# Ighina/MultimodalTopicSegmentation

Hardware: AMD Instinct MI355X
Metric: sentences/sec (fwd+bwd) (higher is better)
Workload: dtype bf16; 1 GPU; BASELINE configs[1]: restricted-window transformer tagger d=1792 heads=8 ff=256 radius=15 layers=1 focal loss, 64 docs x 256 sentences per GPU, fwd+bwd+Adam(eps 1e-7), inputs resident in HBM; global_batch_docs=64, sentences_per_doc=256, parallelism=dp1 (document-sharded, RCCL all-reduce)

## Files before the change

### multimodaltopicsegmentation_amd/csrc/ffn_fused.hip

```cpp
#include <algorithm>
#include "gemm_common.h"

#define FF_BM 64
#define FF_F 256
#define FF_IMG 32768
#define FF_RING (FF_IMG)
#define FF_A_STAGE (8192 + 32768)
#define FF_B_STAGE 32768
#define FF_LDS (FF_IMG + 4 * FF_B_STAGE)
#ifdef FFN_STAMPS
#define FSTAMP(i) do { const unsigned long long t_ = __builtin_amdgcn_s_memtime(); tacc[i] += t_ - tprev; tprev = t_; } while (0)
#else
#define FSTAMP(i) do { } while (0)
#endif

struct FfnArgs {
  const bf16_t* X;
  const bf16_t* Wa;
  const bf16_t* Wb;
  const float* ba;
  const float* bb;
  const bf16_t* U;
  bf16_t* Uout;
  bf16_t* T;
  bf16_t* Y;
  int M, D, relu;
#ifdef FFN_STAMPS
  unsigned long long* stamps;
#endif
};

__device__ __forceinline__ int ff_col(int j, int n) { return (j >> 1) * 32 + (n >> 2) * 8 + (j & 1) * 4 + (n & 3); }

template <bool PERM>
__device__ __forceinline__ void ff_piece_kmajor(const bf16_t* __restrict__ G, int ld, int row0, int dim, int k0, char* img, int piece, int lane) {
  const int row = piece * 8 + (lane >> 3), pos = lane & 7;
  const int ch = pos ^ ((row >> 1) & 7);
  const int srow = PERM ? (row & ~63) + ff_col((row >> 4) & 3, row & 15) : row;
  const bf16_t* src = G + (size_t)min(row0 + srow, dim - 1) * ld + k0 + ch * 8;
  __builtin_amdgcn_global_load_lds((gptr_t*)src, (lptr_t*)(img + piece * 1024), 16, 0, 0);
}
__device__ __forceinline__ void ff_piece_strided(const bf16_t* __restrict__ G, int ld, int k0, int col0, char* img, int piece, int lane) {
  const int kr = piece * 4 + (lane >> 4), c16 = lane & 15;
  const int ch = ((((c16 >> 1) ^ strided_key(kr))) << 1) | (c16 & 1);
  const bf16_t* src = G + (size_t)(k0 + kr) * ld + col0 + ch * 8;
  __builtin_amdgcn_global_load_lds((gptr_t*)src, (lptr_t*)(img + piece * 1024), 16, 0, 0);
}

__device__ __forceinline__ frag_raw ff_frag_strided(const char* tile, int kbase, int wcol0, int j, int lane) {
  const int r = lane & 15, q = r >> 2, p = r & 3;
  const int col = wcol0 + (j >> 1) * 32 + (j & 1) * 4 + 8 * p;
  const unsigned addr = (unsigned)(uintptr_t)(__attribute__((address_space(3))) const char*)(tile + strided_off(kbase + q, col));
  frag_raw f;
  asm volatile("ds_read_b64_tr_b16 %0, %1" : "=v"(f.lo) : "v"(addr));
  asm volatile("ds_read_b64_tr_b16 %0, %1 offset:1024" : "=v"(f.hi) : "v"(addr));
  return f;
}

#define FF_CWAVES 8
#define FF_LWAVES 4
#define FF_THREADS ((FF_CWAVES + FF_LWAVES) * 64)

template <bool BWD>
__global__ __launch_bounds__(FF_THREADS) void ffn_fused_kernel(const FfnArgs a) {
  constexpr bool WKM = !BWD;
  extern __shared__ __attribute__((aligned(16))) char smem[];
  char* fimg = smem;
  char* ring = smem + FF_RING;
  const int tid = threadIdx.x, lane = tid & 63;
  const int wave = __builtin_amdgcn_readfirstlane(tid >> 6);
  const int bm0 = blockIdx.x * FF_BM;
  const int D = a.D, M = a.M;
  const int nkA = D / 64, nch = D / 256, nB = nch * 4;
#ifdef FFN_STAMPS
  unsigned long long tacc[16] = {0, 0, 0, 0, 0, 0, 0, 0, 0, 0, 0, 0, 0, 0, 0, 0};
  unsigned long long tprev = __builtin_amdgcn_s_memtime();
#define FF_STAMPS_OUT() do { if (a.stamps && lane == 0) for (int i_ = 0; i_ < 16; ++i_) a.stamps[((size_t)blockIdx.x * 12 + wave) * 16 + i_] = tacc[i_]; } while (0)
#else
#define FF_STAMPS_OUT() do { } while (0)
#endif

  if (wave >= FF_CWAVES) {
    const int lw = wave - FF_CWAVES;
    auto dmaA = [&](int kt) {
      char* st = ring + (kt % 3) * FF_A_STAGE;
#pragma unroll
      for (int i = 0; i < 10; ++i) {
        const int q = lw * 10 + i;
        if (q < 8) ff_piece_kmajor<false>(a.X, D, bm0, M, kt * 64, st, q, lane);
        else if constexpr (WKM) ff_piece_kmajor<true>(a.Wa, D, 0, FF_F, kt * 64, st + 8192, q - 8, lane);
        else ff_piece_strided(a.Wa, FF_F, kt * 64, ((q - 8) >> 4) * 128, st + 8192 + ((q - 8) >> 4) * 16384, (q - 8) & 15, lane);
      }
    };
    auto dmaB = [&](int gi) {
      char* st = ring + (gi & 3) * FF_B_STAGE;
      const int c = gi >> 2, kk = gi & 3;
#pragma unroll
      for (int i = 0; i < 8; ++i) {
        const int q = lw * 8 + i;
        if constexpr (WKM) ff_piece_kmajor<true>(a.Wb, FF_F, c * 256, D, kk * 64, st, q, lane);
        else ff_piece_strided(a.Wb, D, kk * 64, c * 256 + (q >> 4) * 128, st + (q >> 4) * 16384, q & 15, lane);
      }
    };
    dmaA(0);
    if (nkA > 1) { dmaA(1); asm volatile("s_waitcnt vmcnt(10)" ::: "memory"); }
    else asm volatile("s_waitcnt vmcnt(0)" ::: "memory");
    __builtin_amdgcn_s_barrier();
#pragma clang loop unroll(disable)
    for (int kt = 0; kt < nkA; ++kt) {
      if (kt + 2 < nkA) { dmaA(kt + 2); FSTAMP(0); asm volatile("s_waitcnt vmcnt(10)" ::: "memory"); }
      else asm volatile("s_waitcnt vmcnt(0)" ::: "memory");
      FSTAMP(3);
      __builtin_amdgcn_s_barrier();
      FSTAMP(4);
    }
    dmaB(0);
    dmaB(1);
    dmaB(2);
    dmaB(3);
    FSTAMP(5);
    asm volatile("s_waitcnt vmcnt(0)" ::: "memory");
    __builtin_amdgcn_s_barrier();
    FSTAMP(6);
#pragma clang loop unroll(disable)
    for (int gi = 0; gi < nB; ++gi) {
      if (gi >= 1 && gi + 3 < nB) { dmaB(gi + 3); FSTAMP(8); asm volatile("s_waitcnt vmcnt(16)" ::: "memory"); }
      else asm volatile("s_waitcnt vmcnt(0)" ::: "memory");
      FSTAMP(11);
      __builtin_amdgcn_s_barrier();
      FSTAMP(12);
    }
    FF_STAMPS_OUT();
    return;
  }

  const int wm = wave >> 2, wn = wave & 3;
  const int r16 = lane & 15, g = lane >> 4;
#ifdef FFN_STAMPS
  int tb = 0;
#endif
  f32x4 acc[2][4];
#pragma unroll
  for (int i = 0; i < 2; ++i)
#pragma unroll
    for (int j = 0; j < 4; ++j) acc[i][j] = (f32x4){0.f, 0.f, 0.f, 0.f};

  const unsigned lds0 = (unsigned)(uintptr_t)(__attribute__((address_space(3))) char*)smem;
  unsigned lk[2];
#pragma unroll
  for (int ks = 0; ks < 2; ++ks) lk[ks] = lds0 + r16 * 128 + (((ks * 4 + g) ^ ((r16 >> 1) & 7)) << 4);
  auto mma_tile = [&](int Aoff, int Boff) {
    LFrag<true> fa[2][2];
    LFrag<WKM> fb[4][2];
#pragma unroll
    for (int ks = 0; ks < 2; ++ks) {
      const unsigned ab = lk[ks] + Aoff + wm * 4096, bb = lk[ks] + Boff + wn * 8192;
#pragma unroll
      for (int j = 0; j < 4; ++j) {
        if constexpr (WKM) asm volatile("ds_read_b128 %0, %1 offset:%2" : "=v"(fb[j][ks].k) : "v"(bb), "n"(j * 2048));
        else fb[j][ks].s = ff_frag_strided(smem + Boff + (wn >> 1) * 16384, ks * 32 + 8 * g, (wn & 1) * 64, j, lane);
      }
#pragma unroll
      for (int i = 0; i < 2; ++i) asm volatile("ds_read_b128 %0, %1 offset:%2" : "=v"(fa[i][ks].k) : "v"(ab), "n"(i * 2048));
    }
    lgkm_wait<0>();
    FSTAMP(tb + 1);
    __builtin_amdgcn_s_setprio(1);
#pragma unroll
    for (int ks = 0; ks < 2; ++ks) {
      bf16x8 vb[4];
#pragma unroll
      for (int j = 0; j < 4; ++j) vb[j] = lfrag_get<WKM>(fb[j][ks]);
#pragma unroll
      for (int i = 0; i < 2; ++i) {
        const bf16x8 va = lfrag_get<true>(fa[i][ks]);
#pragma unroll
        for (int j = 0; j < 4; ++j) acc[i][j] = __builtin_amdgcn_mfma_f32_16x16x32_bf16(vb[j], va, acc[i][j], 0, 0, 0);
      }
    }
    __builtin_amdgcn_s_setprio(0);
    FSTAMP(tb + 2);
  };

  typedef __attribute__((ext_vector_type(4))) unsigned u32x4;
  uint4 upre[2][2];
  float4 b1[2][2];
  if constexpr (BWD) {
#pragma unroll
    for (int i = 0; i < 2; ++i)
#pragma unroll
      for (int h = 0; h < 2; ++h)
        upre[i][h] = *reinterpret_cast<const uint4*>(a.U + (size_t)min(bm0 + wm * 32 + i * 16 + r16, M - 1) * FF_F + wn * 64 + h * 32 + g * 8);
  } else {
#pragma unroll
    for (int h = 0; h < 2; ++h)
#pragma unroll
      for (int e = 0; e < 2; ++e) b1[h][e] = *reinterpret_cast<const float4*>(a.ba + wn * 64 + h * 32 + g * 8 + e * 4);
  }
  __builtin_amdgcn_s_barrier();
#pragma clang loop unroll(disable)
  for (int kt = 0; kt < nkA; ++kt) {
    FSTAMP(0);
    const int st = FF_RING + (kt % 3) * FF_A_STAGE;
    mma_tile(st, st + 8192);
    FSTAMP(3);
    __builtin_amdgcn_s_barrier();
    FSTAMP(4);
  }
#pragma unroll
  for (int i = 0; i < 2; ++i) {
    const int row = wm * 32 + i * 16 + r16;
#pragma unroll
    for (int h = 0; h < 2; ++h) {
      float v[8];
#pragma unroll
      for (int e = 0; e < 4; ++e) { v[e] = acc[i][2 * h][e]; v[4 + e] = acc[i][2 * h + 1][e]; }
      const size_t go = (size_t)(bm0 + row) * FF_F + wn * 64 + h * 32 + g * 8;
      if constexpr (!BWD) {
        v[0] += b1[h][0].x; v[1] += b1[h][0].y; v[2] += b1[h][0].z; v[3] += b1[h][0].w;
        v[4] += b1[h][1].x; v[5] += b1[h][1].y; v[6] += b1[h][1].z; v[7] += b1[h][1].w;
        uint4 pre;
        pre.x = pack_bf16x2(v[0], v[1]); pre.y = pack_bf16x2(v[2], v[3]); pre.z = pack_bf16x2(v[4], v[5]); pre.w = pack_bf16x2(v[6], v[7]);
        *reinterpret_cast<uint4*>(a.Uout + go) = pre;
#pragma unroll
        for (int r = 0; r < 8; ++r) v[r] = a.relu ? fmaxf(v[r], 0.0f) : gelu_erf_f(v[r]);
      } else {
        const unsigned uw[4] = {upre[i][h].x, upre[i][h].y, upre[i][h].z, upre[i][h].w};
#pragma unroll
        for (int r = 0; r < 8; ++r) {
          const float uu = (r & 1) ? bf16_hi(uw[r >> 1]) : bf16_lo(uw[r >> 1]);
          const float dr = to_f32(from_f32<bf16_t>(v[r]));
          v[r] = a.relu ? (uu > 0.0f ? dr : 0.0f) : dr * gelu_erf_grad_f(uu);
        }
      }
      uint4 t;
      t.x = pack_bf16x2(v[0], v[1]); t.y = pack_bf16x2(v[2], v[3]); t.z = pack_bf16x2(v[4], v[5]); t.w = pack_bf16x2(v[6], v[7]);
      *reinterpret_cast<uint4*>(a.T + go) = t;
      *reinterpret_cast<uint4*>(fimg + wn * 8192 + kmajor_off(row, h * 4 + g)) = t;
    }
#pragma unroll
    for (int j = 0; j < 4; ++j) acc[i][j] = (f32x4){0.f, 0.f, 0.f, 0.f};
  }
  FSTAMP(5);
  asm volatile("s_waitcnt lgkmcnt(0)" ::: "memory");
  __builtin_amdgcn_s_barrier();
  FSTAMP(6);
#ifdef FFN_STAMPS
  tb = 8;
#endif

  float4 b2[2][2];
  uint4 res[2][2];
#pragma clang loop unroll(disable)
  for (int c = 0; c < nch; ++c) {
    const int colw = c * 256 + wn * 64 + g * 8;
#pragma unroll
    for (int kk = 0; kk < 4; ++kk) {
      const int gi = c * 4 + kk;
      if (kk == 3) {
        if constexpr (!BWD) {
#pragma unroll
          for (int h = 0; h < 2; ++h)
#pragma unroll
            for (int e = 0; e < 2; ++e) b2[h][e] = *reinterpret_cast<const float4*>(a.bb + colw + h * 32 + e * 4);
        }
      }
      if (kk == 1) {
#pragma unroll
        for (int i = 0; i < 2; ++i)
#pragma unroll
          for (int h = 0; h < 2; ++h)
            res[i][h] = *reinterpret_cast<const uint4*>(a.X + (size_t)min(bm0 + wm * 32 + i * 16 + r16, M - 1) * D + colw + h * 32);
      }
      FSTAMP(8);
      mma_tile(kk * 8192, FF_RING + kk * FF_B_STAGE);
      if (kk == 3) {
#pragma unroll
        for (int i = 0; i < 2; ++i) {
          const int row = bm0 + wm * 32 + i * 16 + r16;
#pragma unroll
          for (int h = 0; h < 2; ++h) {
            float v[8];
#pragma unroll
            for (int e = 0; e < 4; ++e) { v[e] = acc[i][2 * h][e]; v[4 + e] = acc[i][2 * h + 1][e]; }
            if constexpr (!BWD) {
              v[0] += b2[h][0].x; v[1] += b2[h][0].y; v[2] += b2[h][0].z; v[3] += b2[h][0].w;
              v[4] += b2[h][1].x; v[5] += b2[h][1].y; v[6] += b2[h][1].z; v[7] += b2[h][1].w;
            }
            const unsigned rw[4] = {res[i][h].x, res[i][h].y, res[i][h].z, res[i][h].w};
#pragma unroll
            for (int e = 0; e < 4; ++e) { v[2 * e] += bf16_lo(rw[e]); v[2 * e + 1] += bf16_hi(rw[e]); }
            uint4 o;
            o.x = pack_bf16x2(v[0], v[1]); o.y = pack_bf16x2(v[2], v[3]); o.z = pack_bf16x2(v[4], v[5]); o.w = pack_bf16x2(v[6], v[7]);
            *reinterpret_cast<uint4*>(a.Y + (size_t)row * D + colw + h * 32) = o;
          }
#pragma unroll
          for (int j = 0; j < 4; ++j) acc[i][j] = (f32x4){0.f, 0.f, 0.f, 0.f};
        }
      }
      FSTAMP(11);
      __builtin_amdgcn_s_barrier();
      FSTAMP(12);
    }
  }
  FF_STAMPS_OUT();
}

#ifdef FFN_STAMPS
static unsigned long long* g_ffn_stamps = nullptr;
extern "C" void mts_ffn_set_stamps(void* p) { g_ffn_stamps = (unsigned long long*)p; }
#endif
static int ffn_launch(bool bwd, hipStream_t st, const FfnArgs& a0) {
  FfnArgs a = a0;
#ifdef FFN_STAMPS
  a.stamps = g_ffn_stamps;
#endif
  const int grid = ceil_div(a.M, FF_BM);
  if (bwd) {
    auto k = ffn_fused_kernel<true>;
    if (int rc = mts_dyn_lds(k, FF_LDS, "ffn_fused")) return rc;
    hipLaunchKernelGGL(k, dim3(grid), dim3(FF_THREADS), FF_LDS, st, a);
  } else {
    auto k = ffn_fused_kernel<false>;
    if (int rc = mts_dyn_lds(k, FF_LDS, "ffn_fused")) return rc;
    hipLaunchKernelGGL(k, dim3(grid), dim3(FF_THREADS), FF_LDS, st, a);
  }
  MTS_LAUNCH_CHECK("mts_ffn_fused");
  return MTS_OK;
}

static int ffn_check(const char* who, int M, int D, int F, const void* p0, const void* p1, const void* p2, const void* p3, const void* p4) {
  MTS_CHECK_ARG(M > 0 && p0 && p1 && p2 && p3 && p4, "%s: bad arguments", who);
  MTS_UNSUPPORTED(F == FF_F && D >= 256 && D % 256 == 0, "%s: the fused block covers F = 256 and D a multiple of 256 (F=%d, D=%d)", who, F, D);
  return MTS_OK;
}

extern "C" int mts_ffn_supported(int dtype, int M, int D, int F) { return dtype == MTS_BF16 && M > 0 && F == FF_F && D >= 256 && D % 256 == 0; }

extern "C" int mts_ffn_fwd(void* stream, int M, int D, int F, const void* a1, const void* w1, const float* b1, const void* w2, const float* b2,
                           int relu, void* u, void* f, void* s2) {
  if (int rc = ffn_check("mts_ffn_fwd", M, D, F, a1, w1, w2, s2, f)) return rc;
  MTS_CHECK_ARG(b1 && b2 && u, "mts_ffn_fwd: null bias / u");
  FfnArgs a{(const bf16_t*)a1, (const bf16_t*)w1, (const bf16_t*)w2, b1, b2, nullptr, (bf16_t*)u, (bf16_t*)f, (bf16_t*)s2, M, D, relu};
  return ffn_launch(false, (hipStream_t)stream, a);
}

extern "C" int mts_ffn_bwd_data(void* stream, int M, int D, int F, const void* ds2, const void* w1, const void* w2, const void* u, int relu,
                                void* du, void* da1) {
  if (int rc = ffn_check("mts_ffn_bwd_data", M, D, F, ds2, w1, w2, du, da1)) return rc;
  MTS_CHECK_ARG(u, "mts_ffn_bwd_data: null u");
  FfnArgs a{(const bf16_t*)ds2, (const bf16_t*)w2, (const bf16_t*)w1, nullptr, nullptr, (const bf16_t*)u, nullptr, (bf16_t*)du, (bf16_t*)da1, M, D, relu};
  return ffn_launch(true, (hipStream_t)stream, a);
}
```

### multimodaltopicsegmentation_amd/csrc/gemm.hip

```cpp
#include <algorithm>
#include <math.h>
#include <stdlib.h>
#include "common.h"

#include "gemm_common.h"


template <int LAYOUT, typename TC, bool GLDS>
__global__ __launch_bounds__(256, 2) void gemm_bf16_kernel(const GemmArgs a) {
  constexpr bool A_KMAJOR = (LAYOUT == MTS_NT || LAYOUT == MTS_NN);
  constexpr bool B_KMAJOR = (LAYOUT == MTS_NT || LAYOUT == MTS_TT);
  extern __shared__ __attribute__((aligned(16))) char smem[];

  const int tid = threadIdx.x;
  const int lane = tid & 63;
  const int wave = tid >> 6;
  const int wm = wave >> 1, wn = wave & 1;
  const int r16 = lane & 15, g = lane >> 4;

  const int ntn = (a.N + BN - 1) / BN;
  const int ntm = (a.M + BM - 1) / BM;
  const int nt = ntn * ntm;
  int bid = xcd_remap(blockIdx.x, nt);
  const int bm0 = (ntm < ntn ? bid % ntm : bid / ntn) * BM;
// ... 329 lines not shown
      float v[4] = {0.f, 0.f, 0.f, 0.f};
      if (kc) {
        const int row = r0 + (f >> 2), k = k0 + (f & 3) * 4;
        if (row < rdim) {
          const float* p = X + (long)row * sr + k;
          if (vec && k + 3 < kend) { const float4 t = *reinterpret_cast<const float4*>(p); v[0] = t.x; v[1] = t.y; v[2] = t.z; v[3] = t.w; }
          else for (int j = 0; j < 4; ++j) if (k + j < kend) v[j] = p[j];
        }
      } else {
        const int k = k0 + (f >> 5), row = r0 + (f & 31) * 4;
        if (k < kend) {
          const float* p = X + (long)k * sk + row;
          if (vec && row + 3 < rdim) { const float4 t = *reinterpret_cast<const float4*>(p); v[0] = t.x; v[1] = t.y; v[2] = t.z; v[3] = t.w; }
          else for (int j = 0; j < 4; ++j) if (row + j < rdim) v[j] = p[j];
        }
      }
      r[i] = make_float4(v[0], v[1], v[2], v[3]);
    }
  };
  auto store_op = [&](float (&S)[F32_BK][F32_PITCH], bool kc, const float4 (&r)[2]) {
#pragma unroll
    for (int i = 0; i < 2; ++i) {
      const int f = tid + 256 * i;
      if (kc) {
        const int row = f >> 2, k = (f & 3) * 4;
        S[k][row] = r[i].x; S[k + 1][row] = r[i].y; S[k + 2][row] = r[i].z; S[k + 3][row] = r[i].w;
      } else {
        *reinterpret_cast<float4*>(&S[f >> 5][(f & 31) * 4]) = r[i];
      }
    }
  };

  f32x4 acc[4][4];
#pragma unroll
  for (int i = 0; i < 4; ++i)
#pragma unroll
    for (int j = 0; j < 4; ++j) acc[i][j] = (f32x4){0.f, 0.f, 0.f, 0.f};

  const int nk = (kend - kbeg + F32_BK - 1) / F32_BK;
  load_op(A, s.sam, s.sak, a_kc, a_vec, bm0, a.M, kbeg, ra);
  load_op(B, s.sbn, s.sbk, b_kc, b_vec, bn0, a.N, kbeg, rb);
  store_op(As[0], a_kc, ra);
  store_op(Bs[0], b_kc, rb);
  __syncthreads();
  for (int kt = 0; kt < nk; ++kt) {
    const int buf = kt & 1;
    if (kt + 1 < nk) {
      load_op(A, s.sam, s.sak, a_kc, a_vec, bm0, a.M, kbeg + (kt + 1) * F32_BK, ra);
      load_op(B, s.sbn, s.sbk, b_kc, b_vec, bn0, a.N, kbeg + (kt + 1) * F32_BK, rb);
    }
#pragma unroll
    for (int ks = 0; ks < F32_BK / 4; ++ks) {
      float av[4], bv[4];
#pragma unroll
      for (int i = 0; i < 4; ++i) {
        av[i] = As[buf][ks * 4 + g][wm * 64 + i * 16 + r16];
        bv[i] = Bs[buf][ks * 4 + g][wn * 64 + i * 16 + r16];
      }
#pragma unroll
      for (int i = 0; i < 4; ++i)
#pragma unroll
        for (int j = 0; j < 4; ++j) acc[i][j] = __builtin_amdgcn_mfma_f32_16x16x4f32(bv[j], av[i], acc[i][j], 0, 0, 0);
    }
    if (kt + 1 < nk) {
      store_op(As[buf ^ 1], a_kc, ra);
      store_op(Bs[buf ^ 1], b_kc, rb);
    }
    __syncthreads();
  }
#pragma unroll
  for (int i = 0; i < 4; ++i) {
    const int m = bm0 + wm * 64 + i * 16 + r16;
#pragma unroll
    for (int j = 0; j < 4; ++j) {
      const int n = bn0 + wn * 64 + j * 16 + 4 * g;
      float v[4] = {acc[i][j][0], acc[i][j][1], acc[i][j][2], acc[i][j][3]};
      epilogue4<float, float>(a, m, n, v, true);
    }
  }
}

#define COLSUM_RS 128
template <typename T>
__global__ __launch_bounds__(256) void colsum_partial_kernel(const T* __restrict__ X, int M, int N, int ldx,
                                                             float* __restrict__ partial) {
  __shared__ float red[16][64];
  const int cx = threadIdx.x & 15, ry = threadIdx.x >> 4;
  const int n = blockIdx.x * 64 + cx * 4;
  const int rs = blockIdx.y;
  const int rows_per = (M + COLSUM_RS - 1) / COLSUM_RS;
  const int m0 = rs * rows_per, m1 = min(M, m0 + rows_per);
  float s[4] = {0.f, 0.f, 0.f, 0.f};
  if (n + 3 < N) {
    int m = m0 + ry;
    for (; m + 48 < m1; m += 64) {
      float v[4][4];
#pragma unroll
      for (int u = 0; u < 4; ++u) load4<T>(X + (size_t)(m + 16 * u) * ldx + n, v[u]);
#pragma unroll
      for (int u = 0; u < 4; ++u)
#pragma unroll
        for (int i = 0; i < 4; ++i) s[i] += v[u][i];
    }
    for (; m < m1; m += 16) {
      float v[4];
      load4<T>(X + (size_t)m * ldx + n, v);
#pragma unroll
      for (int i = 0; i < 4; ++i) s[i] += v[i];
    }
  } else if (n < N) {
    for (int m = m0 + ry; m < m1; m += 16)
      for (int i = 0; i < 4 && n + i < N; ++i) s[i] += to_f32(X[(size_t)m * ldx + n + i]);
  }
#pragma unroll
  for (int i = 0; i < 4; ++i) red[ry][cx * 4 + i] = s[i];
  __syncthreads();
  if (threadIdx.x < 64) {
    const int c = threadIdx.x, nn = blockIdx.x * 64 + c;
    float t = 0.f;
#pragma unroll
    for (int r = 0; r < 16; ++r) t += red[r][c];
    if (nn < N) partial[(size_t)rs * N + nn] = t;
  }
}
__global__ __launch_bounds__(256) void colsum_final_kernel(const float* __restrict__ partial, int N, int nparts,
                                                           float* __restrict__ out, int accumulate) {
  __shared__ float red[4][64];
  const int col = threadIdx.x & 63, grp = threadIdx.x >> 6;
  const int n = blockIdx.x * 64 + col;
  float s = 0.f;
  if (n < N) {
    int r = grp;
    for (; r + 4 * 7 < nparts; r += 4 * 8) {
      float v[8];
#pragma unroll
      for (int u = 0; u < 8; ++u) v[u] = partial[(size_t)(r + 4 * u) * N + n];
#pragma unroll
      for (int u = 0; u < 8; ++u) s += v[u];
    }
    for (; r < nparts; r += 4) s += partial[(size_t)r * N + n];
  }
  red[grp][col] = s;
  __syncthreads();
  if (grp == 0 && n < N) {
    const float t = (red[0][col] + red[1][col]) + (red[2][col] + red[3][col]);
    out[n] = accumulate ? out[n] + t : t;
  }
}

__global__ __launch_bounds__(256) void splitk_reduce_kernel(const float* __restrict__ slab, int splits, int M, int N, float* __restrict__ C,
                                                            int ldc, int accumulate) {
  const size_t idx = (size_t)blockIdx.x * 256 + threadIdx.x;
  const int n4 = N / 4;
  if (idx >= (size_t)M * n4) return;
  const int m = (int)(idx / n4), n = 4 * (int)(idx % n4);
  float s[4] = {0.f, 0.f, 0.f, 0.f};
  if (accumulate) load4<float>(C + (size_t)m * ldc + n, s);
  const size_t plane = (size_t)M * N;
  for (int z = 0; z < splits; ++z) {
    float v[4];
    load4<float>(slab + z * plane + (size_t)m * N + n, v);
#pragma unroll
    for (int i = 0; i < 4; ++i) s[i] += v[i];
  }
  store4<float>(C + (size_t)m * ldc + n, s);
}

__global__ __launch_bounds__(256) void splitk_reduce_t_kernel(const float* __restrict__ slab, int splits, int M, int N, float* __restrict__ Ct,
                                                              int ldc, int accumulate) {
  __shared__ float tile[32][33];
  const int n0 = blockIdx.x * 32, m0 = blockIdx.y * 32;
  const int tx = threadIdx.x & 31, ty = threadIdx.x >> 5;
  const size_t plane = (size_t)M * N;
#pragma unroll
  for (int r = ty; r < 32; r += 8) {
    const int m = m0 + r, n = n0 + tx;
    float s = 0.f;
    if (m < M && n < N) {
      const float* p = slab + (size_t)m * N + n;
      int z = 0;
      for (; z + 7 < splits; z += 8) {
        float v[8];
#pragma unroll
        for (int u = 0; u < 8; ++u) v[u] = p[(size_t)(z + u) * plane];
#pragma unroll
        for (int u = 0; u < 8; ++u) s += v[u];
      }
      for (; z < splits; ++z) s += p[(size_t)z * plane];
    }
    tile[r][tx] = s;
  }
  __syncthreads();
#pragma unroll
  for (int r = ty; r < 32; r += 8) {
    const int n = n0 + r, m = m0 + tx;
    if (n < N && m < M) {
      float* o = Ct + (size_t)n * ldc + m;
      *o = accumulate ? *o + tile[tx][r] : tile[tx][r];
    }
  }
}

template <typename T> __global__ void cast_kernel(const float* __restrict__ src, T* __restrict__ dst, size_t n) {
  size_t i = ((size_t)blockIdx.x * blockDim.x + threadIdx.x) * 4;
  const size_t stride = (size_t)gridDim.x * blockDim.x * 4;
  for (; i + 3 < n; i += stride) {
    float v[4];
    load4<float>(src + i, v);
    store4<T>(dst + i, v);
  }
  if (i < n && i + 3 >= n)
    for (size_t j = i; j < n; ++j) dst[j] = from_f32<T>(src[j]);
}

template <typename T> __global__ void cast_concat_kernel(const float* __restrict__ s1, const float* __restrict__ s2, T* __restrict__ dst,
                                                          size_t rows, int D1, int D2) {
  const int D = D1 + D2, q = D / 4;
  const size_t total = rows * q;
  for (size_t i = (size_t)blockIdx.x * blockDim.x + threadIdx.x; i < total; i += (size_t)gridDim.x * blockDim.x) {
    const size_t r = i / q;
    const int e = (int)(i - r * q) * 4;
    float v[4];
    load4<float>(e < D1 ? s1 + r * D1 + e : s2 + r * D2 + (e - D1), v);
    store4<T>(dst + r * D + e, v);
  }
}

extern "C" int mts_cast_concat(void* stream, int dst_dtype, size_t rows, int D1, int D2, const float* src1, const float* src2, void* dst) {
  MTS_CHECK_ARG(src1 && src2 && dst && D1 > 0 && D2 > 0 && D1 % 4 == 0 && D2 % 4 == 0, "mts_cast_concat: bad arguments (widths must be multiples of 4)");
  if (rows == 0) return MTS_OK;
  const int blocks = (int)std::min<size_t>(4096, (rows * ((D1 + D2) / 4) + 255) / 256);
  if (dst_dtype == MTS_BF16) hipLaunchKernelGGL(cast_concat_kernel<bf16_t>, dim3(blocks), dim3(256), 0, (hipStream_t)stream, src1, src2, (bf16_t*)dst, rows, D1, D2);
  else if (dst_dtype == MTS_F32) hipLaunchKernelGGL(cast_concat_kernel<float>, dim3(blocks), dim3(256), 0, (hipStream_t)stream, src1, src2, (float*)dst, rows, D1, D2);
  else { mts_set_error("mts_cast_concat: bad dtype %d", dst_dtype); return MTS_ERR_INVALID; }
  MTS_LAUNCH_CHECK("mts_cast_concat");
  return MTS_OK;
}

extern "C" size_t mts_colsum_workspace(int N) { return (size_t)COLSUM_RS * (size_t)N * sizeof(float); }

extern "C" int mts_colsum(void* stream, int dtype, int M, int N, const void* X, int ldx, float* out, int accumulate,
                          void* partial) {
  MTS_CHECK_ARG(M > 0 && N > 0 && X && out && partial, "mts_colsum: bad arguments");
  MTS_CHECK_ARG(dtype == MTS_F32 || dtype == MTS_BF16, "mts_colsum: bad dtype %d", dtype);
  MTS_CHECK_ARG(ldx % 4 == 0, "mts_colsum: ldx must be a multiple of 4");
  hipStream_t st = (hipStream_t)stream;
  const int nparts = min(COLSUM_RS, M);
  dim3 grid(ceil_div(N, 64), COLSUM_RS);
  (void)nparts;
  if (dtype == MTS_F32)
    hipLaunchKernelGGL(colsum_partial_kernel<float>, grid, dim3(256), 0, st, (const float*)X, M, N, ldx, (float*)partial);
  else
    hipLaunchKernelGGL(colsum_partial_kernel<bf16_t>, grid, dim3(256), 0, st, (const bf16_t*)X, M, N, ldx, (float*)partial);
  hipLaunchKernelGGL(colsum_final_kernel, dim3(ceil_div(N, 64)), dim3(256), 0, st, (const float*)partial, N, COLSUM_RS, out,
                     accumulate);
  MTS_LAUNCH_CHECK("mts_colsum");
  return MTS_OK;
}

extern "C" int mts_cast(void* stream, int dst_dtype, const float* src, void* dst, size_t n) {
  MTS_CHECK_ARG(src && dst, "mts_cast: null pointer");
  if (n == 0) return MTS_OK;
  hipStream_t st = (hipStream_t)stream;
  const int blocks = (int)std::min<size_t>(2048, (n / 4 + 255) / 256 + 1);
  if (dst_dtype == MTS_BF16)
    hipLaunchKernelGGL(cast_kernel<bf16_t>, dim3(blocks), dim3(256), 0, st, src, (bf16_t*)dst, n);
  else if (dst_dtype == MTS_F32)
    hipLaunchKernelGGL(cast_kernel<float>, dim3(blocks), dim3(256), 0, st, src, (float*)dst, n);
  else {
    mts_set_error("mts_cast: bad dtype %d", dst_dtype);
    return MTS_ERR_INVALID;
  }
  MTS_LAUNCH_CHECK("mts_cast");
  return MTS_OK;
}

int mts_launch_gemm256(const GemmArgs& a, int layout, bool c_is_f32, int splits, hipStream_t st);
int mts_launch_gemm224(const GemmArgs& a, int layout, bool c_is_f32, int splits, hipStream_t st);
bool mts_gemm224t_applies(const GemmArgs& a, int layout, bool c_is_f32, int splits);

static thread_local int g_gemm_glds = -1;
static thread_local int g_tile_mode = -1;
static thread_local int g_force_splits = 0;
static thread_local int g_tile_order = 1;
static thread_local int g_gemm_deep = 1;
static thread_local int g_chain = 0;
static thread_local int g_combine = 0;
#define MTS_GEMM_WS_HEAD 8192
static thread_local int g_last_tile = 0, g_last_splits = 0;

static thread_local void (*g_mid_hook)(void) = nullptr;
extern "C" int mts_gemm_set_mid_hook(void (*fn)(void)) { g_mid_hook = fn; return MTS_OK; }

extern "C" int mts_gemm_last_plan(int* tile, int* splits) {
  if (tile) *tile = g_last_tile;
  if (splits) *splits = g_last_splits;
  return MTS_OK;
}

void mts_band_set_mfma(int on);
void mts_band_set_fused(int on);
void mts_full_set_mfma(int on);
void mts_t5_set_mfma(int on);
static thread_local int g_f32_mfma = 1;
static thread_local int g_big_min_k = 256;
static thread_local int g_gemm_variant = 0;
void mts_lstm_pair_set_spin_limit(int n);
void mts_lstm_pair_set_max_pairs(int n);
void mts_lstm_pair_set_parts(int n);
extern "C" int mts_set_option(const char* key, int value) {
  if (!key) return MTS_ERR_INVALID;
  if (!strcmp(key, "gemm_tile")) { g_tile_mode = value; return MTS_OK; }
  if (!strcmp(key, "gemm_glds")) { g_gemm_glds = value; return MTS_OK; }
  if (!strcmp(key, "gemm_splits")) { g_force_splits = value; return MTS_OK; }
  if (!strcmp(key, "gemm_order")) { g_tile_order = value; return MTS_OK; }
  if (!strcmp(key, "gemm_chain")) { g_chain = value; return MTS_OK; }
  if (!strcmp(key, "gemm_combine")) { g_combine = value; return MTS_OK; }
  if (!strcmp(key, "gemm_deep")) { g_gemm_deep = value; return MTS_OK; }
  if (!strcmp(key, "gemm_variant")) { g_gemm_variant = value; return MTS_OK; }
  if (!strcmp(key, "gemm_big_min_k")) { g_big_min_k = value; return MTS_OK; }
  if (!strcmp(key, "gemm_f32_mfma")) { g_f32_mfma = value; return MTS_OK; }
  if (!strcmp(key, "band_mfma")) { mts_band_set_mfma(value); return MTS_OK; }
  if (!strcmp(key, "band_fused_bwd")) { mts_band_set_fused(value); return MTS_OK; }
  if (!strcmp(key, "full_mfma")) { mts_full_set_mfma(value); return MTS_OK; }
  if (!strcmp(key, "t5_mfma")) { mts_t5_set_mfma(value); return MTS_OK; }
  if (!strcmp(key, "lstm_pair_spin_limit")) { mts_lstm_pair_set_spin_limit(value); return MTS_OK; }
  if (!strcmp(key, "lstm_pair_max_pairs")) { mts_lstm_pair_set_max_pairs(value); return MTS_OK; }
  if (!strcmp(key, "lstm_parts")) { mts_lstm_pair_set_parts(value); return MTS_OK; }
  mts_set_error("mts_set_option: unknown key %s", key);
  return MTS_ERR_INVALID;
}

template <int LAYOUT, typename TC>
static void launch_bf16(const GemmArgs& a, int splits, hipStream_t st) {
  const int nt = ceil_div(a.M, BM) * ceil_div(a.N, BN);
  if (g_gemm_glds < 0) {
    const char* e = getenv("MTS_GEMM_GLDS");
    g_gemm_glds = (e && e[0] == '0') ? 0 : 1;
  }
  const bool glds = g_gemm_glds && (a.K % BK == 0) && (a.ksplit % BK == 0) && a.M >= 8 && a.N >= 8;
  if (glds) {
    GemmArgs b = a;
    const bool deep = g_gemm_deep && (size_t)nt * splits <= 256 && a.ksplit >= 4 * BK;
    b.nbuf = deep ? 4 : 2;
    auto k = gemm_bf16_kernel<LAYOUT, TC, true>;
    if (deep && mts_dyn_lds(k, 8 * TILE_BYTES, "gemm") != MTS_OK) b.nbuf = 2;
    hipLaunchKernelGGL(k, dim3(nt, 1, splits), dim3(256), (b.nbuf == 4 ? 8 : 4) * TILE_BYTES, st, b);
  } else {
    hipLaunchKernelGGL((gemm_bf16_kernel<LAYOUT, TC, false>), dim3(nt, 1, splits), dim3(256), 4 * TILE_BYTES, st, a);
  }
}

static void plan_bf16(int c_dtype, int layout, int M, int N, int K, unsigned epilogue, bool has_workspace, size_t workspace_bytes,
                      int* use256_out, int* splits_out) {
  if (g_tile_mode < 0) {
    const char* e = getenv("MTS_GEMM_TILE");
    g_tile_mode = e ? atoi(e) : 0;
  }
  const int tile_mode = g_tile_mode;
  const unsigned plain = epilogue & ~MTS_EPI_ACCUM;
  const bool can_split = (c_dtype == MTS_F32 && plain == 0 && has_workspace && N % 4 == 0 && K >= 2048);
  const bool can256 = (K % BK == 0) && K >= g_big_min_k && M >= 8 && N >= 8 && tile_mode != 128;
  const double bw = 3500.0;
  double best = 1e30;
  int splits = 1;
  int use256 = 0;
  const bool can224 = can256 && (N % 224 == 0) && tile_mode != 256;
  for (int big = 0; big <= (can256 ? 2 : 0); ++big) {
    if (big == 2 && !can224) continue;
    if (tile_mode == 256 && can256 && big != 1) continue;
    if (tile_mode == 224 && can224 && big != 2) continue;
    const int tile = big ? 256 : 128;
    const double slots = big ? 256.0 : 512.0;
    const double t_k = layout == MTS_TN ? (big == 2 ? (M % 256 == 0 ? 0.0160 : 0.0200) : big == 1 ? 0.0218 : 0.0145)
                                        : (big ? 0.0232 * (big == 2 ? 0.875 : 1.0) : 0.0180);
    const double t_0 = big ? 7.7 : 6.5;
    const int nt = ceil_div(M, tile) * (big == 2 ? N / 224 : ceil_div(N, tile));
    for (int sp = 1; sp <= (can_split ? 32 : 1); ++sp) {
      const int ks = ceil_div(ceil_div(K, sp), BK) * BK;
      if (ceil_div(K, ks) != sp) continue;
      if (sp > 1 && (size_t)sp * M * N * sizeof(float) > workspace_bytes) break;
      if (g_force_splits > 0 && can_split && sp != g_force_splits) continue;
      const double rounds = ceil((double)nt * sp / slots);
      const double cost = rounds * (ks * t_k + t_0) + (sp > 1 ? (2.0 * sp + 1.0) * M * N * 4.0 / 1e6 / bw : 0.0);
      if (cost < best) { best = cost; splits = sp; use256 = big; }
    }
  }
  *use256_out = use256;
  *splits_out = splits;
}

int mts_gemm224_last_kernel();
int mts_launch_gemm224t_pair(const GemmArgs& a, int splits, const void* A2, const void* B2, float* slab2, hipStream_t st);
bool mts_gemm224t_applies(const GemmArgs& a, int layout, bool c_is_f32, int splits);

static int wgrad_pair_splits(int M, int N, int K, size_t workspace_bytes) {
  if (M % 256 || N % 224 || K % 64 || K < 256) return -1;
  static int cus = 0;
  if (!cus) { int dev = 0; hipDeviceProp_t pr; cus = (hipGetDevice(&dev) == hipSuccess && hipGetDeviceProperties(&pr, dev) == hipSuccess) ? pr.multiProcessorCount : 256; }
  const int nt = (M / 256) * (N / 224);
  int sp = std::max(1, std::min(32, cus / (2 * nt)));
  for (; sp >= 1; --sp) {
    const int ks = ceil_div(ceil_div(K, sp), BK) * BK;
    if (ceil_div(K, ks) != sp) continue;
    if (ks >= 128 && K - (sp - 1) * ks >= 128 && (size_t)2 * sp * M * N * sizeof(float) <= workspace_bytes) return sp;
  }
  return -1;
}
extern "C" size_t mts_wgrad_pair_workspace(int M, int N, int K) {
  const int sp = wgrad_pair_splits(M, N, K, (size_t)-1);
  return sp < 1 ? 0 : (size_t)2 * sp * M * N * sizeof(float);
}
extern "C" int mts_wgrad_pair(void* stream, int M, int N, int K, const void* A1, const void* B1, float* C1, int ldc1, const void* A2, const void* B2,
                              float* C2t, int ldc2t, int lda, int ldb, int accumulate, void* workspace, size_t workspace_bytes) {
  MTS_CHECK_ARG(M > 0 && N > 0 && K > 0 && A1 && B1 && C1 && A2 && B2 && C2t && workspace, "mts_wgrad_pair: bad arguments");
  MTS_CHECK_ARG(ldc1 >= N && ldc2t >= M && ldc1 % 4 == 0, "mts_wgrad_pair: bad output strides");
  const int sp = wgrad_pair_splits(M, N, K, workspace_bytes);
  MTS_UNSUPPORTED(sp >= 1, "mts_wgrad_pair: M=%d N=%d K=%d not covered (M %% 256, N %% 224, K %% 64) or workspace too small", M, N, K);
  hipStream_t st = (hipStream_t)stream;
  GemmArgs a;
  memset(&a, 0, sizeof(a));
  a.A = A1; a.B = B1; a.C = C1;
  a.M = M; a.N = N; a.K = K; a.lda = lda; a.ldb = ldb; a.ldc = ldc1;
  a.epi = 0; a.colscale = 1.0f;
  a.ksplit = ceil_div(ceil_div(K, sp), BK) * BK;
  a.order = 1; a.nbuf = 2; a.variant = 0;
  float* const planes = (float*)workspace;
  a.slab = planes;
  float* const planes2 = planes + (size_t)sp * M * N;
  MTS_UNSUPPORTED(mts_gemm224t_applies(a, MTS_TN, true, sp), "mts_wgrad_pair: operands not covered by the four-wave weight-gradient kernel (alignment / strides)");
  const int rc = mts_launch_gemm224t_pair(a, sp, A2, B2, planes2, st);
  MTS_UNSUPPORTED(rc == MTS_OK, "mts_wgrad_pair: launch refused");
  hipLaunchKernelGGL(splitk_reduce_kernel, dim3((unsigned)(((size_t)M * (N / 4) + 255) / 256)), dim3(256), 0, st, (const float*)planes, sp, M, N, C1, ldc1,
                     accumulate ? 1 : 0);
  hipLaunchKernelGGL(splitk_reduce_t_kernel, dim3(ceil_div(N, 32), ceil_div(M, 32)), dim3(256), 0, st, (const float*)planes2, sp, M, N, C2t, ldc2t,
                     accumulate ? 1 : 0);
  MTS_LAUNCH_CHECK("mts_wgrad_pair");
  return MTS_OK;
}

extern "C" int mts_gemm_plan(int a_dtype, int c_dtype, int layout, int M, int N, int K, unsigned epilogue, size_t workspace_bytes,
                             int* tile, int* splits) {
  MTS_CHECK_ARG(M > 0 && N > 0 && K > 0, "mts_gemm_plan: bad shape M=%d N=%d K=%d", M, N, K);
  MTS_CHECK_ARG(layout == MTS_NT || layout == MTS_NN || layout == MTS_TN || layout == MTS_TT, "mts_gemm_plan: bad layout %d", layout);
  MTS_CHECK_ARG(a_dtype == MTS_F32 || a_dtype == MTS_BF16, "mts_gemm_plan: bad a_dtype %d", a_dtype);
  int use256 = 0, sp = 1;
  const size_t ws_planes = workspace_bytes > MTS_GEMM_WS_HEAD ? workspace_bytes - MTS_GEMM_WS_HEAD : 0;
  if (a_dtype == MTS_BF16) plan_bf16(c_dtype, layout, M, N, K, epilogue, ws_planes > 0, ws_planes, &use256, &sp);
  if (tile) *tile = a_dtype == MTS_F32 ? (g_f32_mfma ? 128 : 64) : use256 == 2 ? 224 : use256 == 1 ? 256 : 128;
  if (splits) *splits = sp;
  return MTS_OK;
}

extern "C" int mts_gemm(void* stream, int a_dtype, int c_dtype, int layout, int M, int N, int K, const void* A, int lda,
                        const void* B, int ldb, void* C, int ldc, const float* bias, const void* residual, int ldr,
                        void* aux, int ldaux, unsigned epilogue, float colscale, int ncols_scaled, void* workspace, size_t workspace_bytes) {
  MTS_CHECK_ARG(M > 0 && N > 0 && K > 0, "mts_gemm: bad shape M=%d N=%d K=%d", M, N, K);
  MTS_CHECK_ARG(A && B && C, "mts_gemm: null operand");
  MTS_CHECK_ARG(layout == MTS_NT || layout == MTS_NN || layout == MTS_TN || layout == MTS_TT, "mts_gemm: bad layout %d", layout);
  MTS_CHECK_ARG(a_dtype == MTS_F32 || a_dtype == MTS_BF16, "mts_gemm: bad a_dtype %d", a_dtype);
  MTS_CHECK_ARG(c_dtype == MTS_F32 || c_dtype == a_dtype, "mts_gemm: c_dtype must be f32 or a_dtype");
  MTS_CHECK_ARG(!(epilogue & MTS_EPI_BIAS) || bias, "mts_gemm: MTS_EPI_BIAS without bias");
  MTS_CHECK_ARG(!(epilogue & MTS_EPI_RESIDUAL) || residual, "mts_gemm: MTS_EPI_RESIDUAL without residual");
  MTS_CHECK_ARG(!(epilogue & MTS_EPI_ACCUM) || c_dtype == MTS_F32, "mts_gemm: MTS_EPI_ACCUM needs fp32 C");
  MTS_CHECK_ARG((epilogue & (MTS_EPI_GELU | MTS_EPI_RELU)) != (MTS_EPI_GELU | MTS_EPI_RELU), "mts_gemm: MTS_EPI_GELU and MTS_EPI_RELU are exclusive");
  hipStream_t st = (hipStream_t)stream;
  GemmArgs a;
  a.A = A; a.B = B; a.C = C; a.bias = bias; a.residual = residual; a.aux = aux;
  a.M = M; a.N = N; a.K = K; a.lda = lda; a.ldb = ldb; a.ldc = ldc; a.ldr = ldr; a.ldaux = ldaux;
  a.epi = epilogue; a.colscale = colscale; a.ncols_scaled = ncols_scaled;
  a.variant = g_gemm_variant;
#ifdef MTS_GEMM_STAMPS
  a.stamps = nullptr;
#endif
  a.ksplit = K; a.slab = nullptr; a.chain = nullptr; a.order = g_tile_order; a.nbuf = 2;

  if (a_dtype == MTS_F32) {
    StrideArgs s;
    if (layout == MTS_NT) { s.sam = lda; s.sak = 1; s.sbn = ldb; s.sbk = 1; }
    else if (layout == MTS_NN) { s.sam = lda; s.sak = 1; s.sbn = 1; s.sbk = ldb; }
    else if (layout == MTS_TT) { s.sam = 1; s.sak = lda; s.sbn = ldb; s.sbk = 1; }
    else { s.sam = 1; s.sak = lda; s.sbn = 1; s.sbk = ldb; }
    MTS_CHECK_ARG(ldc % 4 == 0 && ((uintptr_t)C % 16) == 0, "mts_gemm(f32): C must be 16-byte aligned with ldc %% 4 == 0");
    MTS_CHECK_ARG(!(epilogue & MTS_EPI_RESIDUAL) || (ldr % 4 == 0 && ((uintptr_t)residual % 16) == 0), "mts_gemm(f32): residual must be 16-byte aligned with ldr %% 4 == 0");
    MTS_CHECK_ARG(!aux || (ldaux % 4 == 0 && ((uintptr_t)aux % 16) == 0), "mts_gemm(f32): aux must be 16-byte aligned with ldaux %% 4 == 0");
    const int nt = ceil_div(M, F32_BM) * ceil_div(N, F32_BM);
    int splits = 1;
    if (g_f32_mfma && workspace && !(epilogue & ~MTS_EPI_ACCUM) && N % 4 == 0 && nt <= 128 && K >= 1024) {
      splits = std::min(std::min(16, 256 / nt), K / 512);
      while (splits > 1 && (size_t)splits * M * N * sizeof(float) > workspace_bytes) --splits;
    }
    g_last_tile = 128;
    g_last_splits = splits;
    if (splits > 1) {
      a.ksplit = ceil_div(ceil_div(K, splits), F32_BK) * F32_BK;
      splits = ceil_div(K, a.ksplit);
      a.slab = (float*)workspace;
    }
    if (g_f32_mfma) hipLaunchKernelGGL(gemm_f32_mfma_kernel, dim3(nt, 1, splits), dim3(256), 0, st, a, s);
    else hipLaunchKernelGGL(gemm_f32_kernel, dim3(ceil_div(M, 64) * ceil_div(N, 64)), dim3(256), 0, st, a, s);
    if (splits > 1)
      hipLaunchKernelGGL(splitk_reduce_kernel, dim3((unsigned)(((size_t)M * (N / 4) + 255) / 256)), dim3(256), 0, st, (const float*)workspace,
                         splits, M, N, (float*)C, ldc, (epilogue & MTS_EPI_ACCUM) ? 1 : 0);
    MTS_LAUNCH_CHECK("mts_gemm(f32)");
    return MTS_OK;
  }

  MTS_UNSUPPORTED(lda % 8 == 0 && ldb % 8 == 0 && ((uintptr_t)A % 16) == 0 && ((uintptr_t)B % 16) == 0,
                  "mts_gemm(bf16): A/B must be 16-byte aligned with ld %% 8 == 0 (lda=%d ldb=%d)", lda, ldb);
  if (layout == MTS_NT) MTS_UNSUPPORTED(K % 8 == 0, "mts_gemm(bf16,NT): K %% 8 != 0 (K=%d)", K);
  if (layout == MTS_NN) MTS_UNSUPPORTED(K % 8 == 0 && N % 8 == 0, "mts_gemm(bf16,NN): K,N %% 8 (K=%d N=%d)", K, N);
  if (layout == MTS_TN) MTS_UNSUPPORTED(M % 8 == 0 && N % 8 == 0, "mts_gemm(bf16,TN): M,N %% 8 (M=%d N=%d)", M, N);
  if (layout == MTS_TT) MTS_UNSUPPORTED(M % 8 == 0 && K % 8 == 0, "mts_gemm(bf16,TT): M,K %% 8 (M=%d K=%d)", M, K);
  MTS_UNSUPPORTED(ldc % 4 == 0 && ((uintptr_t)C % (c_dtype == MTS_F32 ? 16 : 8)) == 0, "mts_gemm(bf16): C alignment/ldc");
  MTS_UNSUPPORTED(!(epilogue & MTS_EPI_RESIDUAL) || (ldr % 4 == 0 && ((uintptr_t)residual % 8) == 0), "mts_gemm(bf16): residual alignment");
  MTS_UNSUPPORTED(!aux || (ldaux % 4 == 0 && ((uintptr_t)aux % 8) == 0), "mts_gemm(bf16): aux alignment");

  int splits = 1, use256 = 0;
  const size_t ws_planes = workspace_bytes > MTS_GEMM_WS_HEAD ? workspace_bytes - MTS_GEMM_WS_HEAD : 0;
  float* const planes = workspace ? (float*)((char*)workspace + MTS_GEMM_WS_HEAD) : nullptr;
  plan_bf16(c_dtype, layout, M, N, K, epilogue, workspace != nullptr && ws_planes > 0, ws_planes, &use256, &splits);
  if (use256 && c_dtype != MTS_F32 && ((uintptr_t)C % 16) != 0) use256 = 0;
  g_last_tile = use256 == 2 ? 224 : use256 == 1 ? 256 : 128;
  g_last_splits = splits;
  a.slab = nullptr;
  bool chained = false;
  if (splits > 1) {
    a.ksplit = ceil_div(ceil_div(K, splits), BK) * BK;
    chained = g_chain && !use256;
    if (chained) {
      const size_t nt128 = (size_t)ceil_div(M, BM) * ceil_div(N, BN);
      a.chain = (unsigned*)planes;
      hipError_t e = hipMemsetAsync(planes, 0, nt128 * sizeof(unsigned), st);
      if (e != hipSuccess) { mts_set_error("mts_gemm: hipMemsetAsync: %s", hipGetErrorString(e)); return MTS_ERR_LAUNCH; }
    } else {
      a.slab = planes;
      if (use256 == 2 && g_combine && (a.variant == 0 || a.variant == 11 || a.variant == 12) && (size_t)ceil_div(M, 256) * (N / 224) * sizeof(unsigned) <= MTS_GEMM_WS_HEAD &&
          mts_gemm224t_applies(a, layout, c_dtype == MTS_F32, splits)) {
        a.chain = (unsigned*)workspace;
        chained = true;
      }
    }
  }
  if (use256) {
    int rc = use256 == 2 ? mts_launch_gemm224(a, layout, c_dtype == MTS_F32, splits, st) : mts_launch_gemm256(a, layout, c_dtype == MTS_F32, splits, st);
    if (rc) return rc;
    if (use256 == 2) g_last_tile = mts_gemm224_last_kernel();
  } else if (c_dtype == MTS_F32) {
    if (layout == MTS_NT) launch_bf16<MTS_NT, float>(a, splits, st);
    else if (layout == MTS_NN) launch_bf16<MTS_NN, float>(a, splits, st);
    else if (layout == MTS_TT) launch_bf16<MTS_TT, float>(a, splits, st);
    else launch_bf16<MTS_TN, float>(a, splits, st);
  } else {
    if (layout == MTS_NT) launch_bf16<MTS_NT, bf16_t>(a, splits, st);
    else if (layout == MTS_NN) launch_bf16<MTS_NN, bf16_t>(a, splits, st);
    else if (layout == MTS_TT) launch_bf16<MTS_TT, bf16_t>(a, splits, st);
    else launch_bf16<MTS_TN, bf16_t>(a, splits, st);
  }
  if (g_mid_hook) g_mid_hook();
  if (splits > 1 && !chained)
    hipLaunchKernelGGL(splitk_reduce_kernel, dim3((unsigned)(((size_t)M * (N / 4) + 255) / 256)), dim3(256), 0, st, (const float*)planes,
                       splits, M, N, (float*)C, ldc, (epilogue & MTS_EPI_ACCUM) ? 1 : 0);
  MTS_LAUNCH_CHECK("mts_gemm(bf16)");
  return MTS_OK;
}
```

Baseline: 9.415 million sentences/s.

## Software-pipeline LDS fragment reads across barriers in fused FFN and pair-swap epilogue stores

Adds a PIPE variant of the fused FFN kernel, enabled by default. Each step prefetches the next k-step's LDS fragments while the MFMAs for the current one run, using a single barrier per step so LDS read latency overlaps compute. The second GEMM drops its per-chunk trailing barrier. Epilogue global stores of Uout/T/Y and the residual/U loads are rearranged via a DPP lane-pair swap so each lane writes a contiguous 64-byte row segment. This costs more registers for the double-buffered fragments and makes the barrier removal's correctness depend on the ring staging.

Result: no change. 9.433 million sentences/s, median of 4 (+0.2%).

```diff
diff --git a/multimodaltopicsegmentation_amd/csrc/ffn_fused.hip b/multimodaltopicsegmentation_amd/csrc/ffn_fused.hip
--- a/multimodaltopicsegmentation_amd/csrc/ffn_fused.hip
+++ b/multimodaltopicsegmentation_amd/csrc/ffn_fused.hip
@@ -32,6 +32,14 @@
 
 __device__ __forceinline__ int ff_col(int j, int n) { return (j >> 1) * 32 + (n >> 2) * 8 + (j & 1) * 4 + (n & 3); }
 
+__device__ __forceinline__ void ff_pair_swap(uint4& p0, uint4& p1, bool odd) {
+#define FF_SWAP1(m) do { const unsigned s_ = odd ? p0.m : p1.m; \
+    const unsigned r_ = (unsigned)__builtin_amdgcn_mov_dpp((int)s_, 0xB1, 0xF, 0xF, true);       \
+    p0.m = odd ? r_ : p0.m; p1.m = odd ? p1.m : r_; } while (0)
+  FF_SWAP1(x); FF_SWAP1(y); FF_SWAP1(z); FF_SWAP1(w);
+#undef FF_SWAP1
+}
+
 template <bool PERM>
 __device__ __forceinline__ void ff_piece_kmajor(const bf16_t* __restrict__ G, int ld, int row0, int dim, int k0, char* img, int piece, int lane) {
   const int row = piece * 8 + (lane >> 3), pos = lane & 7;
@@ -61,7 +69,7 @@
 #define FF_LWAVES 4
 #define FF_THREADS ((FF_CWAVES + FF_LWAVES) * 64)
 
-template <bool BWD>
+template <bool BWD, bool PIPE>
 __global__ __launch_bounds__(FF_THREADS) void ffn_fused_kernel(const FfnArgs a) {
   constexpr bool WKM = !BWD;
   extern __shared__ __attribute__((aligned(16))) char smem[];
@@ -182,7 +190,48 @@
     FSTAMP(tb + 2);
   };
 
+  constexpr int NR = 4 * lfrag_ops<WKM>::value + 2;
+  LFrag<true> fa[2][2];
+  LFrag<WKM> fb[4][2];
+  auto rd = [&](const int ks, int Aoff, int Boff) __attribute__((always_inline)) {
+    const unsigned ab = lk[ks] + Aoff + wm * 4096, bb = lk[ks] + Boff + wn * 8192;
+#pragma unroll
+    for (int j = 0; j < 4; ++j) {
+      if constexpr (WKM) asm volatile("ds_read_b128 %0, %1 offset:%2" : "=v"(fb[j][ks].k) : "v"(bb), "n"(j * 2048));
+      else fb[j][ks].s = ff_frag_strided(smem + Boff + (wn >> 1) * 16384, ks * 32 + 8 * g, (wn & 1) * 64, j, lane);
+    }
+#pragma unroll
+    for (int i = 0; i < 2; ++i) asm volatile("ds_read_b128 %0, %1 offset:%2" : "=v"(fa[i][ks].k) : "v"(ab), "n"(i * 2048));
+  };
+  auto mm = [&](const int ks) __attribute__((always_inline)) {
+    __builtin_amdgcn_s_setprio(1);
+    bf16x8 vb[4];
+#pragma unroll
+    for (int j = 0; j < 4; ++j) vb[j] = lfrag_get<WKM>(fb[j][ks]);
+#pragma unroll
+    for (int i = 0; i < 2; ++i) {
+      const bf16x8 va = lfrag_get<true>(fa[i][ks]);
+#pragma unroll
+      for (int j = 0; j < 4; ++j) acc[i][j] = __builtin_amdgcn_mfma_f32_16x16x32_bf16(vb[j], va, acc[i][j], 0, 0, 0);
+    }
+    __builtin_amdgcn_s_setprio(0);
+  };
+  auto pstep = [&](int Aoff, int Boff, const bool nxt, int nA, int nB_) __attribute__((always_inline)) {
+    rd(1, Aoff, Boff);
+    lgkm_wait<NR>();
+    mm(0);
+    lgkm_wait<0>();
+    FSTAMP(tb + 2);
+    __builtin_amdgcn_s_barrier();
+    FSTAMP(tb + 4);
+    if (nxt) rd(0, nA, nB_);
+    mm(1);
+  };
+
   typedef __attribute__((ext_vector_type(4))) unsigned u32x4;
+  const bool odd = r16 & 1;
+  auto erow = [&](int t) { return PIPE ? (r16 & ~1) + t : r16; };
+  auto ehalf = [&](int t) { return PIPE ? (int)odd : t; };
   uint4 upre[2][2];
   float4 b1[2][2];
   if constexpr (BWD) {
@@ -190,7 +239,7 @@
     for (int i = 0; i < 2; ++i)
 #pragma unroll
       for (int h = 0; h < 2; ++h)
-        upre[i][h] = *reinterpret_cast<const uint4*>(a.U + (size_t)min(bm0 + wm * 32 + i * 16 + r16, M - 1) * FF_F + wn * 64 + h * 32 + g * 8);
+        upre[i][h] = *reinterpret_cast<const uint4*>(a.U + (size_t)min(bm0 + wm * 32 + i * 16 + erow(h), M - 1) * FF_F + wn * 64 + ehalf(h) * 32 + g * 8);
   } else {
 #pragma unroll
     for (int h = 0; h < 2; ++h)
@@ -198,6 +247,18 @@
       for (int e = 0; e < 2; ++e) b1[h][e] = *reinterpret_cast<const float4*>(a.ba + wn * 64 + h * 32 + g * 8 + e * 4);
   }
   __builtin_amdgcn_s_barrier();
+  if constexpr (PIPE) {
+    FSTAMP(4);
+    rd(0, FF_RING, FF_RING + 8192);
+    int st = FF_RING;
+#pragma clang loop unroll(disable)
+    for (int kt = 0; kt + 1 < nkA; ++kt) {
+      const int stn = (kt % 3 == 2) ? FF_RING : st + FF_A_STAGE;
+      pstep(st, st + 8192, true, stn, stn + 8192);
+      st = stn;
+    }
+    pstep(st, st + 8192, false, 0, 0);
+  } else {
 #pragma clang loop unroll(disable)
   for (int kt = 0; kt < nkA; ++kt) {
     FSTAMP(0);
@@ -207,9 +268,12 @@
     __builtin_amdgcn_s_barrier();
     FSTAMP(4);
   }
+  }
 #pragma unroll
   for (int i = 0; i < 2; ++i) {
     const int row = wm * 32 + i * 16 + r16;
+    uint4 po[2], to[2];
+    if constexpr (PIPE && BWD) ff_pair_swap(upre[i][0], upre[i][1], odd);
 #pragma unroll
     for (int h = 0; h < 2; ++h) {
       float v[8];
@@ -221,7 +285,8 @@
         v[4] += b1[h][1].x; v[5] += b1[h][1].y; v[6] += b1[h][1].z; v[7] += b1[h][1].w;
         uint4 pre;
         pre.x = pack_bf16x2(v[0], v[1]); pre.y = pack_bf16x2(v[2], v[3]); pre.z = pack_bf16x2(v[4], v[5]); pre.w = pack_bf16x2(v[6], v[7]);
-        *reinterpret_cast<uint4*>(a.Uout + go) = pre;
+        if constexpr (PIPE) po[h] = pre;
+        else *reinterpret_cast<uint4*>(a.Uout + go) = pre;
 #pragma unroll
         for (int r = 0; r < 8; ++r) v[r] = a.relu ? fmaxf(v[r], 0.0f) : gelu_erf_f(v[r]);
       } else {
@@ -235,8 +300,19 @@
       }
       uint4 t;
       t.x = pack_bf16x2(v[0], v[1]); t.y = pack_bf16x2(v[2], v[3]); t.z = pack_bf16x2(v[4], v[5]); t.w = pack_bf16x2(v[6], v[7]);
-      *reinterpret_cast<uint4*>(a.T + go) = t;
+      if constexpr (PIPE) to[h] = t;
+      else *reinterpret_cast<uint4*>(a.T + go) = t;
       *reinterpret_cast<uint4*>(fimg + wn * 8192 + kmajor_off(row, h * 4 + g)) = t;
+    }
+    if constexpr (PIPE) {
+      if constexpr (!BWD) ff_pair_swap(po[0], po[1], odd);
+      ff_pair_swap(to[0], to[1], odd);
+#pragma unroll
+      for (int t = 0; t < 2; ++t) {
+        const size_t go = (size_t)(bm0 + wm * 32 + i * 16 + erow(t)) * FF_F + wn * 64 + ehalf(t) * 32 + g * 8;
+        if constexpr (!BWD) *reinterpret_cast<uint4*>(a.Uout + go) = po[t];
+        *reinterpret_cast<uint4*>(a.T + go) = to[t];
+      }
     }
 #pragma unroll
     for (int j = 0; j < 4; ++j) acc[i][j] = (f32x4){0.f, 0.f, 0.f, 0.f};
@@ -251,6 +327,7 @@
 
   float4 b2[2][2];
   uint4 res[2][2];
+  if constexpr (PIPE) rd(0, 0, FF_RING);
 #pragma clang loop unroll(disable)
   for (int c = 0; c < nch; ++c) {
     const int colw = c * 256 + wn * 64 + g * 8;
@@ -270,14 +347,21 @@
         for (int i = 0; i < 2; ++i)
 #pragma unroll
           for (int h = 0; h < 2; ++h)
-            res[i][h] = *reinterpret_cast<const uint4*>(a.X + (size_t)min(bm0 + wm * 32 + i * 16 + r16, M - 1) * D + colw + h * 32);
-      }
+            res[i][h] = *reinterpret_cast<const uint4*>(a.X + (size_t)min(bm0 + wm * 32 + i * 16 + erow(h), M - 1) * D + colw + ehalf(h) * 32);
+      }
+      if constexpr (PIPE) {
+        const int kn = (kk + 1) & 3;
+        pstep(kk * 8192, FF_RING + kk * FF_B_STAGE, true, kn * 8192, FF_RING + kn * FF_B_STAGE);
+      } else {
       FSTAMP(8);
       mma_tile(kk * 8192, FF_RING + kk * FF_B_STAGE);
+      }
       if (kk == 3) {
 #pragma unroll
         for (int i = 0; i < 2; ++i) {
           const int row = bm0 + wm * 32 + i * 16 + r16;
+          uint4 yo[2];
+          if constexpr (PIPE) ff_pair_swap(res[i][0], res[i][1], odd);
 #pragma unroll
           for (int h = 0; h < 2; ++h) {
             float v[8];
@@ -292,15 +376,24 @@
             for (int e = 0; e < 4; ++e) { v[2 * e] += bf16_lo(rw[e]); v[2 * e + 1] += bf16_hi(rw[e]); }
             uint4 o;
             o.x = pack_bf16x2(v[0], v[1]); o.y = pack_bf16x2(v[2], v[3]); o.z = pack_bf16x2(v[4], v[5]); o.w = pack_bf16x2(v[6], v[7]);
-            *reinterpret_cast<uint4*>(a.Y + (size_t)row * D + colw + h * 32) = o;
+            if constexpr (PIPE) yo[h] = o;
+            else *reinterpret_cast<uint4*>(a.Y + (size_t)row * D + colw + h * 32) = o;
+          }
+          if constexpr (PIPE) {
+            ff_pair_swap(yo[0], yo[1], odd);
+#pragma unroll
+            for (int t = 0; t < 2; ++t)
+              *reinterpret_cast<uint4*>(a.Y + (size_t)(bm0 + wm * 32 + i * 16 + erow(t)) * D + colw + ehalf(t) * 32) = yo[t];
           }
 #pragma unroll
           for (int j = 0; j < 4; ++j) acc[i][j] = (f32x4){0.f, 0.f, 0.f, 0.f};
         }
       }
+      if constexpr (!PIPE) {
       FSTAMP(11);
       __builtin_amdgcn_s_barrier();
       FSTAMP(12);
+      }
     }
   }
   FF_STAMPS_OUT();
@@ -310,23 +403,28 @@
 static unsigned long long* g_ffn_stamps = nullptr;
 extern "C" void mts_ffn_set_stamps(void* p) { g_ffn_stamps = (unsigned long long*)p; }
 #endif
+static thread_local int g_ffn_variant = 0;
+void mts_ffn_set_variant(int v) { g_ffn_variant = v; }
+#ifdef FFN_STAMPS
+extern "C" void mts_ffn_stamps_variant(int v) { g_ffn_variant = v; }
+#endif
+
+template <bool BWD, bool PIPE>
+static int ffn_launch_as(hipStream_t st, const FfnArgs& a) {
+  auto k = ffn_fused_kernel<BWD, PIPE>;
+  if (int rc = mts_dyn_lds(k, FF_LDS, "ffn_fused")) return rc;
+  hipLaunchKernelGGL(k, dim3(ceil_div(a.M, FF_BM)), dim3(FF_THREADS), FF_LDS, st, a);
+  MTS_LAUNCH_CHECK("mts_ffn_fused");
+  return MTS_OK;
+}
 static int ffn_launch(bool bwd, hipStream_t st, const FfnArgs& a0) {
   FfnArgs a = a0;
 #ifdef FFN_STAMPS
   a.stamps = g_ffn_stamps;
 #endif
-  const int grid = ceil_div(a.M, FF_BM);
-  if (bwd) {
-    auto k = ffn_fused_kernel<true>;
-    if (int rc = mts_dyn_lds(k, FF_LDS, "ffn_fused")) return rc;
-    hipLaunchKernelGGL(k, dim3(grid), dim3(FF_THREADS), FF_LDS, st, a);
-  } else {
-    auto k = ffn_fused_kernel<false>;
-    if (int rc = mts_dyn_lds(k, FF_LDS, "ffn_fused")) return rc;
-    hipLaunchKernelGGL(k, dim3(grid), dim3(FF_THREADS), FF_LDS, st, a);
-  }
-  MTS_LAUNCH_CHECK("mts_ffn_fused");
-  return MTS_OK;
+  const bool pipe = g_ffn_variant != 1;
+  if (bwd) return pipe ? ffn_launch_as<true, true>(st, a) : ffn_launch_as<true, false>(st, a);
+  return pipe ? ffn_launch_as<false, true>(st, a) : ffn_launch_as<false, false>(st, a);
 }
 
 static int ffn_check(const char* who, int M, int D, int F, const void* p0, const void* p1, const void* p2, const void* p3, const void* p4) {
diff --git a/multimodaltopicsegmentation_amd/csrc/gemm.hip b/multimodaltopicsegmentation_amd/csrc/gemm.hip
--- a/multimodaltopicsegmentation_amd/csrc/gemm.hip
+++ b/multimodaltopicsegmentation_amd/csrc/gemm.hip
@@ -655,6 +655,7 @@
 void mts_band_set_fused(int on);
 void mts_full_set_mfma(int on);
 void mts_t5_set_mfma(int on);
+void mts_ffn_set_variant(int v);
 static thread_local int g_f32_mfma = 1;
 static thread_local int g_big_min_k = 256;
 static thread_local int g_gemm_variant = 0;
@@ -677,6 +678,7 @@
   if (!strcmp(key, "band_fused_bwd")) { mts_band_set_fused(value); return MTS_OK; }
   if (!strcmp(key, "full_mfma")) { mts_full_set_mfma(value); return MTS_OK; }
   if (!strcmp(key, "t5_mfma")) { mts_t5_set_mfma(value); return MTS_OK; }
+  if (!strcmp(key, "ffn_variant")) { mts_ffn_set_variant(value); return MTS_OK; }
   if (!strcmp(key, "lstm_pair_spin_limit")) { mts_lstm_pair_set_spin_limit(value); return MTS_OK; }
   if (!strcmp(key, "lstm_pair_max_pairs")) { mts_lstm_pair_set_max_pairs(value); return MTS_OK; }
   if (!strcmp(key, "lstm_parts")) { mts_lstm_pair_set_parts(value); return MTS_OK; }
```
